# ifpen/wfcrl-env

Measured on AMD Instinct MI355X. Metric: farm_steps_per_sec, higher is better.
Workload: dtype f32

## Files before the change

### wfcrl-env_amd/csrc/wf_kernels_ll.hip

```cpp
#include <hip/hip_runtime.h>

#include <cstring>
#include <mutex>
#include <type_traits>
#include <utility>

#include "wf_kernel_common.h"

#ifndef WF_LL_PART
#define WF_LL_PART 0
#endif

namespace {

template <class F, int... I>
__device__ __forceinline__ void static_for_impl(F&& f, std::integer_sequence<int, I...>) {
  (f(std::integral_constant<int, I>{}), ...);
}
template <int N, class F>
__device__ __forceinline__ void static_for(F&& f) {
  static_for_impl(f, std::make_integer_sequence<int, N>{});
}

__device__ __forceinline__ void sincos_yaw(float x, float& s, float& c) {
  const float x2 = x * x;
  s = x * fmaf(x2, fmaf(x2, fmaf(x2, fmaf(x2, 2.7557319e-6f, -1.9841270e-4f), 8.3333333e-3f), -1.6666667e-1f), 1.0f);
  c = fmaf(x2, fmaf(x2, fmaf(x2, fmaf(x2, fmaf(x2, -2.7557319e-7f, 2.4801587e-5f), -1.3888889e-3f), 4.1666667e-2f), -0.5f), 1.0f);
  if (__any(fabsf(x) > 0.8f)) {
    float s2, c2;
    sincosf(x, &s2, &c2);
    s = (fabsf(x) > 0.8f) ? s2 : s;
    c = (fabsf(x) > 0.8f) ? c2 : c;
  }
}

template <int G>
__device__ __forceinline__ float wave_max(float v) {
  auto dpp = [](float x, auto ctrl, auto rows) {
    return __int_as_float(__builtin_amdgcn_update_dpp(__float_as_int(x), __float_as_int(x), decltype(ctrl)::value, decltype(rows)::value, 0xf, false));
  };
  using I = std::integral_constant<int, 0>;
  (void)sizeof(I);
  if constexpr (G < 2) v = fmaxf(v, dpp(v, std::integral_constant<int, 0xB1>{}, std::integral_constant<int, 0xf>{}));
  if constexpr (G < 4) v = fmaxf(v, dpp(v, std::integral_constant<int, 0x4E>{}, std::integral_constant<int, 0xf>{}));
  if constexpr (G < 8) v = fmaxf(v, dpp(v, std::integral_constant<int, 0x141>{}, std::integral_constant<int, 0xf>{}));
  if constexpr (G < 16) v = fmaxf(v, dpp(v, std::integral_constant<int, 0x140>{}, std::integral_constant<int, 0xf>{}));
  v = fmaxf(v, dpp(v, std::integral_constant<int, 0x142>{}, std::integral_constant<int, 0xa>{}));
  v = fmaxf(v, dpp(v, std::integral_constant<int, 0x143>{}, std::integral_constant<int, 0xc>{}));
  return __int_as_float(__builtin_amdgcn_readlane(__float_as_int(v), 63));
}

template <int G>
__device__ __forceinline__ float sub_max(float v) {
  auto dpp = [](float x, auto ctrl) {
    return __int_as_float(__builtin_amdgcn_update_dpp(__float_as_int(x), __float_as_int(x), decltype(ctrl)::value, 0xf, 0xf, false));
  };
  static_assert(G >= 2 && G <= 8, "sub_max: lanes per farm");
  if constexpr (G < 4) v = fmaxf(v, dpp(v, std::integral_constant<int, 0x4E>{}));
  if constexpr (G < 8) v = fmaxf(v, dpp(v, std::integral_constant<int, 0x124>{}));
  v = fmaxf(v, dpp(v, std::integral_constant<int, 0x128>{}));
  v = fmaxf(v, __shfl_xor(v, 16));
  v = fmaxf(v, __shfl_xor(v, 32));
  return v;
}

template <int G, int OS>
__device__ __forceinline__ float group_bcast(float v, int gbase) {
  if constexpr (G == 2) {
    return __int_as_float(__builtin_amdgcn_update_dpp(__float_as_int(v), __float_as_int(v), OS | (OS << 2) | ((2 + OS) << 4) | ((2 + OS) << 6), 0xf, 0xf, false));
  } else if constexpr (G == 4) {
    return __int_as_float(__builtin_amdgcn_update_dpp(__float_as_int(v), __float_as_int(v), OS * 0x55, 0xf, 0xf, false));
  } else {
    return __shfl(v, gbase + OS);
  }
}

struct SrcLog {
  float Gy, Gwt, sy0d, sz0d;
  float sM, tan_th0, sy0v, snw;
  float kdef, x0d, kyd, pj;
  float x0v, kyv, ch_pref, ix0v;
  float inv_s0d, d0;
};
struct ColdRec { float4 a, b, c; };
static_assert(WF_LOG_HOT_FLOATS == 2 && WF_LOG_COLD_FLOATS == 12, "source log record");
struct WfLogSide { float TI0, TI1, TI2, dTI; };
struct SrcB { float ubar, ct, a, Gwr, Gy, Gwt; unsigned risk; };
struct SrcD { SrcLog Sc; WfLogSide X; bool split; float x0num_d, pfac, b2om_d; };

}

#if WF_LL_PART != 1
__global__ void wf_pair_table_ll_kernel(const WfPairConsts pc, int G, const double* __restrict__ gx,
                                        const double* __restrict__ gy, float* __restrict__ tab, size_t group_floats,
                                        int* __restrict__ cross_tie, int* __restrict__ own_ok, int own_mode, double reach0,
                                        double reach_k) {
  const int i = blockIdx.x, t = threadIdx.x, grp = blockIdx.y;
  const int nblk = (pc.N + G - 1) / G;
  if (t >= nblk * G) return;
  gx += (size_t)grp * pc.N;
  gy += (size_t)grp * pc.N;
  const int J = t / G;
  if (own_mode == 1 && i >= J * G && i < t && t < pc.N) {
    const double dx = gx[t] - gx[i], dy = gy[t] - gy[i];
    if (dx <= 0.0 || fabs(dy) < reach0 + reach_k * dx) own_ok[(size_t)grp * nblk + J] = 0;
  }
  if (i >= (J + 1) * G) {
    if (t < pc.N && gx[t] - gx[i] >= 0.0) atomicOr(&cross_tie[grp], 1);
    return;
  }
  float* o = tab + (size_t)grp * group_floats + wf_ll_block_offset(J, pc.N, G) + ((size_t)i * G + (t - J * G)) * WF_PAIR_STRIDE;
  wf_pair_record(pc, gx, gy, i, t, o);
}

extern "C" size_t wfk_ll_table_floats(int N, int G) { return wf_ll_block_offset((N + G - 1) / G, N, G); }

extern "C" hipError_t wfk_launch_pair_table_ll(const WfPairConsts* pc, int G, int n_groups, const double* gx, const double* gy,
                                               float* tab, int* cross_tie, int* own_ok, int own_mode, double reach0,
                                               double reach_k, hipStream_t s) {
  const int nblk = (pc->N + G - 1) / G;
  const int threads = ((nblk * G + 63) / 64) * 64;
  hipError_t e = hipMemsetAsync(cross_tie, 0, sizeof(int) * (size_t)n_groups, s);
  if (e != hipSuccess) return e;
  e = hipMemsetD32Async((hipDeviceptr_t)own_ok, own_mode ? 1 : 0, (size_t)n_groups * nblk, s);
  if (e != hipSuccess) return e;
  hipLaunchKernelGGL(wf_pair_table_ll_kernel, dim3(pc->N, n_groups), dim3(threads), 0, s, *pc, G, gx, gy, tab,
                     wfk_ll_table_floats(pc->N, G), cross_tie, own_ok, own_mode, reach0, reach_k);
  return hipGetLastError();
}
#else
extern "C" size_t wfk_ll_table_floats(int N, int G);
#endif

#ifdef WF_LL_STAMP
static __device__ unsigned long long wf_ll_stamp[16];
#define WF_T(v) const unsigned long long v = __builtin_readcyclecounter()
#define WF_ACC(k, a, b) st_acc[k] += (b) - (a)
#else
#define WF_T(v)
#define WF_ACC(k, a, b)
#endif
template <int G, int S, bool UWS, bool TAB, bool MC1, int WPB, bool VEER = false, bool OCC2 = false>
__global__ __launch_bounds__(64 * WPB, ((S == 1 && !OCC2) ? 3 : 2) * 4 / WPB) void wf_step_ll_kernel(
    const WfConsts c, const WfTables* __restrict__ tab, const int* __restrict__ gidx, const double* __restrict__ ws_in,
    const double* __restrict__ wd_in, int wind_stride, const float* __restrict__ yaw_in, float* __restrict__ o_power,
    float* __restrict__ o_ws, float* __restrict__ o_wd, float* __restrict__ o_load, int B, const WfEnvArgs ea,
    const float* __restrict__ ll_tab, size_t group_floats, const int* __restrict__ cross_tie, float* __restrict__ src_log,
    size_t log_cold_offset, size_t log_side_offset, int n_pad, const WfGroupArgs ga, const double* __restrict__ gx,
    const double* __restrict__ gy, const int* __restrict__ own_ok) {
  constexpr int EPW = 64 / G;
  constexpr int GS = G * S;
  constexpr int CH = 64 / GS;
  constexpr bool STAGE = TAB && !VEER && GS <= CH;
  constexpr int CHUNK_FLOATS = TAB ? 64 * WF_PAIR_STRIDE : 4;
  __shared__ TableLds T;
  __shared__ __attribute__((aligned(16))) float prow[2][CHUNK_FLOATS];
  __shared__ unsigned risk_lds[WPB][EPW];
  __shared__ int env_lds[WPB][EPW];
  extern __shared__ __attribute__((aligned(16))) float yaw_lds[];

  if (ga.res_zero && blockIdx.x == 0 && threadIdx.x == 0) *ga.res_zero = 0;
  int grp = 0;
  if (ga.blk_group) {
    grp = ga.blk_group[(blockIdx.x * (WPB * EPW)) / ga.blk_unit];
    if (grp < 0) return;
    grp = (grp + ga.shift) % ga.mod;
  }
  if constexpr (TAB) {
    if (cross_tie[grp]) return;
    ll_tab += (size_t)grp * group_floats;
  }

  auto stage_chunk = [&](int q) {
    const char* g0 = reinterpret_cast<const char*>(ll_tab) + (size_t)q * (CHUNK_FLOATS * 4);
    char* l0 = reinterpret_cast<char*>(&prow[q & 1][0]);
    for (int ch = (int)(threadIdx.x >> 6); ch < CHUNK_FLOATS * 4 / 1024; ch += WPB)
      lds_dma16(g0 + ch * 1024 + (threadIdx.x & 63) * 16, l0 + ch * 1024, false);
  };
  if constexpr (TAB) stage_chunk(0);
  for (int k = threadIdx.x; k < WF_TABLE_PAD; k += blockDim.x) {
    T.knot[k] = tab->knot[k];
    T.ct[k] = tab->ct[k];
    T.cts[k] = tab->ct_slope[k];
    T.pw[k] = tab->pw[k];
    T.pws[k] = tab->pw_slope[k];
  }
  for (int k = threadIdx.x; k < WF_BUCKETS; k += blockDim.x) T.bucket[k] = tab->bucket[k];

  const int lane = threadIdx.x & 63;
  const int wave = threadIdx.x >> 6;
  const int sub = lane & (G - 1);
  const int gbase = lane & ~(G - 1);
  const int eiw = lane / G;
  const int slot = (blockIdx.x * WPB + wave) * EPW + eiw;
  int env_raw = slot + ga.env_base;
  if (ga.perm) env_raw = ga.perm[env_raw];
  bool env_ok = env_raw >= 0 && env_raw < (ga.env_end ? ga.env_end : B);
  const int env = env_ok ? env_raw : (B - 1);
  if constexpr (!TAB) env_ok = env_ok && !cross_tie[env];
  if (sub == 0) risk_lds[wave][eiw] = 0u;
  const int N = c.N;
  const int nblk = (N + GS - 1) / GS;

  auto uni = [](float v) { return UWS ? __int_as_float(__builtin_amdgcn_readfirstlane(__float_as_int(v))) : v; };
  const float ws = uni((float)ws_in[(size_t)env * wind_stride]);
  const double wd_d = fmod(wd_in[(size_t)env * wind_stride], 360.0);
  const float wd = uni((float)(wd_d < 0.0 ? wd_d + 360.0 : wd_d));
  const float Ui[3] = {uni(ws * c.shearf[0]), uni(ws * c.shearf[1]), uni(ws * c.shearf[2])};
  const float offk = c.off[2] * kGs;
  const float U02c = uni(Ui[0] * Ui[0] * Ui[0] + Ui[2] * Ui[2] * Ui[2]), U1c = uni(Ui[1] * Ui[1] * Ui[1]);
  auto cube_sum = [&](const float* e) {
    if constexpr (VEER) {
      float m = 0.0f;
#pragma unroll
      for (int j = 0; j < 3; ++j)
#pragma unroll
        for (int k = 0; k < 3; ++k) {
          const float u = Ui[k] * (1.0f - fsqrt(e[3 * j + k]));
          m = fmaf(u * u, u, m);
        }
      return m;
    } else {
      float fe = 0.0f, fc = 0.0f;
#pragma unroll
      for (int j = 0; j < 3; ++j) {
        const float ue = 1.0f - fsqrt(e[2 * j]), uc = 1.0f - fsqrt(e[2 * j + 1]);
        fe = fmaf(ue * ue, ue, fe);
        fc = fmaf(uc * uc, uc, fc);
      }
      return fmaf(U02c, fe, U1c * fc);
    }
  };
  const float ovh = 0.5f * c.guard_inv;
  const float ovs[3] = {uni(ovh * Ui[0] * c.inv_overlap_thr), uni(ovh * Ui[1] * c.inv_overlap_thr), uni(ovh * Ui[2] * c.inv_overlap_thr)};
  const float ovc = 0.5f - ovh;

  const size_t gofs = TAB ? (size_t)grp * N : (size_t)env * N;
  const size_t yofs = (size_t)env * N;
  const bool env_mode = ea.yaw_state != nullptr;
  int moves_new = 0;
  if (env_mode && ea.action) moves_new = ea.moves[env] + 1;
  if (sub == 0) env_lds[wave][eiw] = env_ok ? env : -1 - env;
  if (env_mode && ea.action) {
    int f = 0, o = lane;
    while (o >= N) { o -= N; ++f; }
    while (f < EPW) {
      const int e_raw = env_lds[wave][f];
      const bool okf = e_raw >= 0;
      const int e = okf ? e_raw : -1 - e_raw;
      const size_t oi = (size_t)e * N + o;
      float yw = ea.yaw_state[oi];
      float a = ea.action[oi];
      float acc = ea.acc[oi];
      const float frac = __fdiv_rn(__fdiv_rn(__fdiv_rn(acc, ea.rate), (float)(ea.moves[e] + 1)), ea.dt);
      if (frac >= ea.budget) a = 0.0f;
      if (ea.discrete) a = (a - 1.0f) * ea.yaw_step;
      if (!ea.discrete) a = fminf(fmaxf(a, -ea.yaw_step), ea.yaw_step);
      yw = fminf(fmaxf(yw + a, ea.yaw_lo), ea.yaw_hi);
      acc += fabsf(a);
      if (okf) {
        ea.yaw_state[oi] = yw;
        ea.acc[oi] = acc;
        if (ea.yaw_out) ea.yaw_out[oi] = yw;
      }
      o += 64;
      while (o >= N) { o -= N; ++f; }
    }
  }
  const float* const yaw_src = (env_mode ? ea.yaw_state : yaw_in) + yofs;
  const bool yaw_fresh = env_mode && ea.action;
  auto load_yaw = [&](int o) { return yaw_fresh ? __hip_atomic_load(yaw_src + o, __ATOMIC_RELAXED, __HIP_MEMORY_SCOPE_AGENT) : yaw_src[o]; };
  if (env_mode && ea.action && sub == 0 && env_ok) ea.moves[env] = moves_new;
  if constexpr (TAB) wf_dma_wait();
  __syncthreads();

  constexpr int NE = VEER ? 9 : 6;
  float esq[S][NE], V[S][9], W[S][9], TI[S][3];
  const float amb0 = fsqrt(c.amb2);

  auto apply_tab = [&](auto PP, const float4* pr, float Gy, float Gwt) {
    constexpr int p = decltype(PP)::value;
#pragma unroll
    for (int j = 0; j < 3; ++j) {
      const float4 cf[3] = {pr[3 * j], pr[3 * j + 1], pr[3 * j + 2]};
#pragma unroll
      for (int k = 0; k < 3; ++k) {
        const int q = j * 3 + k;
        V[p][q] = fmaf(Gwt, cf[k].y, fmaf(Gy, cf[k].x, V[p][q]));
        const float ww = fmaf(Gwt, cf[k].w, Gy * cf[k].z);
        W[p][q] += fmaxf(ww, 0.0f);
      }
    }
  };

  auto apply_tab_ratio = [&](auto PP, const float4* pr, float rho, float Gwt) {
    constexpr int p = decltype(PP)::value;
    const float lim = copysignf(__builtin_inff(), Gwt);
#pragma unroll
    for (int q = 0; q < 9; ++q) {
      const float4 cf = pr[q];
      V[p][q] = fmaf(Gwt, fmaf(rho, cf.x, cf.y), V[p][q]);
      W[p][q] = fmaf(Gwt, __builtin_amdgcn_fmed3f(fmaf(rho, cf.z, cf.w), 0.0f, lim), W[p][q]);
    }
  };

  auto apply_fly = [&](auto PP, float dx, float dy, float Gy, float Gwt) {
    constexpr int p = decltype(PP)::value;
    const float Gt = c.gam_top * Gy, Gb = -c.gam_bot * Gy;
    float dec[3];
#pragma unroll
    for (int k = 0; k < 3; ++k) dec[k] = frcp(fmaf(c.decay_a[k], dx, 1.0f));
#pragma unroll
    for (int j = 0; j < 3; ++j) {
      const float yL = dy + c.yoff[j];
      const float yL2 = yL * yL;
      const float Ey = fexp2(-yL2 * c.exp_c);
      float A[3] = {0.0f, 0.0f, 0.0f}, Bw[3] = {0.0f, 0.0f, 0.0f};
#pragma unroll
      for (int mi = 0; mi < 7; ++mi) {
        float tr = fmaf(-Ey, c.ez[mi], 1.0f) * frcp(yL2 + c.zc2[mi]);
        if (mi == 3) {
          const float ts = fmaf(yL2 + c.zc2[3], c.m_half_inv_eps4, c.inv_eps2);
          tr = (yL2 < c.yl2_small) ? ts : tr;
        }
// ... 327 lines not shown
  };
  auto src_far_bound = [&](const SrcD& d, const float* TIs, float& k6, float& b6, float& n6) {
    const SrcLog& Sc = d.Sc;
    const float s0 = VEER ? c.sz0v : Sc.sy0v;
    float kyv_m = Sc.kyv, bb = fmaf(-Sc.kyv, Sc.x0v, s0);
    float db = fabsf(Sc.tan_th0 * Sc.x0d) + 2.2f * fabsf(Sc.pj);
    if (__any(d.split)) {
      const float TImax = fmaxf(TIs[0], fmaxf(TIs[1], TIs[2])), TImin = fminf(TIs[0], fminf(TIs[1], TIs[2]));
      const float x0d_m = d.x0num_d * frcp(fmaf(c.alpha4_d, TImin, d.b2om_d));
      const float pj_m = d.pfac * frcp(fmaf(c.ka_d, TImin, c.kb_d));
      kyv_m = fmaf(c.ka, TImax + d.X.dTI, c.kb);
      bb = d.split ? s0 : bb;
      db = fabsf(Sc.tan_th0 * x0d_m) + 2.2f * fabsf(pj_m);
    }
    const float dbo = db + c.off[2];
    k6 = c.far_k * kyv_m;
    b6 = fmaf(c.far_k, bb, dbo);
    n6 = fmaf(c.far_k, fmaxf(Sc.snw, s0), dbo);
  };
  auto within_bound = [&](const float4 bnd, float dx, float dy) {
    return fabsf(dy) < fmaxf(fmaf(bnd.x, dx, bnd.y), bnd.z) + fabsf(fmaf(c.bd, dx, c.ad));
  };
  int oidx[S], oidx_nx[S], oidx_n2[S];
  float yaw_nx[S];
#pragma unroll
  for (int p = 0; p < S; ++p) {
    oidx_nx[p] = gidx[gofs + min(p * G + sub, N - 1)];
    oidx_n2[p] = gidx[gofs + min(GS + p * G + sub, N - 1)];
  }
#pragma unroll
  for (int p = 0; p < S; ++p) yaw_nx[p] = load_yaw(oidx_nx[p]);
  for (int J = 0; J < nblk; ++J) {
    int tt[S];
    bool tvalid[S];
    float yaw_t[S], sg_t[S], cg_t[S];
    double xt_d[TAB ? 1 : S] = {}, yt_d[TAB ? 1 : S] = {};
#pragma unroll
    for (int p = 0; p < S; ++p) {
      tt[p] = J * GS + p * G + sub;
      tvalid[p] = tt[p] < N;
      if constexpr (!TAB) {
        xt_d[p] = tvalid[p] ? gx[gofs + tt[p]] : -1.0e300;
        yt_d[p] = gy[gofs + (tvalid[p] ? tt[p] : 0)];
      }
#pragma unroll
      for (int k = 0; k < 9; ++k) { V[p][k] = 0.0f; W[p][k] = 0.0f; }
#pragma unroll
      for (int k = 0; k < NE; ++k) esq[p][k] = 0.0f;
#pragma unroll
      for (int j = 0; j < 3; ++j) TI[p][j] = amb0;
      oidx[p] = oidx_nx[p];
      yaw_t[p] = yaw_nx[p];
      oidx_nx[p] = oidx_n2[p];
      oidx_n2[p] = gidx[gofs + min(tt[p] + 2 * GS, N - 1)];
      yaw_nx[p] = load_yaw(oidx_nx[p]);
      sincos_yaw(yaw_t[p] * kDeg2Rad, sg_t[p], cg_t[p]);
    }

    const int first_own = J * GS;
    const int n_src = min(N, first_own + GS);
    const int n_chunks = (n_src + CH - 1) / CH;
    float2 hot_nx = make_float2(0.0f, 0.0f);
    ColdRec cold_nx = {};
    double xs_nx = 0.0, ys_nx = 0.0;
    if (first_own > 0) {
      if constexpr (!TAB) {
        hot_nx = load_hot(0);
        cold_nx = load_cold(0);
        xs_nx = gx[gofs];
        ys_nx = gy[gofs];
      }
    }

    auto fly_record = [&](auto PP, double xi, double yi) {
      constexpr int p = decltype(PP)::value;
      constexpr int q = TAB ? 0 : p;
      float4 r;
      r.x = (float)(xt_d[q] - xi);
      r.y = (float)(yt_d[q] - yi);
      r.z = (xt_d[q] <= xi + c.fifteenD_d) ? 1.0f : 0.0f;
      r.w = __int_as_float((xt_d[q] > xi + 0.1) ? 8 : 0);
      return r;
    };

    auto own_source = [&](auto PS, int i, const float* recs) {
      constexpr int ps = decltype(PS)::value;
      const int src = gbase + ((i - first_own) - ps * G);
      __builtin_amdgcn_s_setprio(3);
      WF_T(so_0);
      float vsum = 0.0f;
#pragma unroll
      for (int k2 = 0; k2 < 9; ++k2) vsum += V[ps][k2];
      const float m3 = __shfl(cube_sum(esq[ps]), src);
      const float Vmean = __shfl(vsum, src) * (1.0f / 9.0f);
      float TIs[3];
#pragma unroll
      for (int j = 0; j < 3; ++j) TIs[j] = __shfl(TI[ps][j], src);
      const float yaw_i = __shfl(yaw_t[ps], src);
      const float cg = __shfl(cg_t[ps], src), sg = __shfl(sg_t[ps], src);
      WF_T(so_1);
      WF_ACC(6, so_0, so_1);
      const SrcB Bs = src_part_b(m3, cg, sg);
      if (Bs.risk) atomicOr(&risk_lds[wave][eiw], Bs.risk);
      WF_T(so_2);
      WF_ACC(7, so_1, so_2);
      float4 ex[S];
      double xi_d = 0.0, yi_d = 0.0;
      if constexpr (!TAB) {
        xi_d = gx[gofs + i];
        yi_d = gy[gofs + i];
      }
      auto pass1_slot = [&](auto PP) {
        constexpr int p = decltype(PP)::value;
        if constexpr (TAB) {
          const float* rec = recs + (p * G + sub) * WF_PAIR_STRIDE;
          ex[p] = *reinterpret_cast<const float4*>(rec + WF_PAIR_DX);
          const bool act1 = (p > ps) ? tvalid[p] : (ex[p].x >= 0.0f);
          if (p >= ps || __any(act1)) {
            if (act1) apply_tab(PP, reinterpret_cast<const float4*>(rec), Bs.Gy, Bs.Gwt);
          }
        } else {
          ex[p] = fly_record(PP, xi_d, yi_d);
          const bool act1 = (p > ps) ? tvalid[p] : (ex[p].x >= 0.0f);
          if (p >= ps || __any(act1)) {
            if (act1) apply_fly(PP, ex[p].x, ex[p].y, Bs.Gy, Bs.Gwt);
          }
        }
      };
      static_for<S>(pass1_slot);
      WF_T(so_3);
      WF_ACC(8, so_2, so_3);
      float vbar = 0.0f, wbar = 0.0f;
#pragma unroll
      for (int k2 = 0; k2 < 9; ++k2) { vbar += V[ps][k2]; wbar += W[ps][k2]; }
      vbar = __shfl(vbar, src) * (1.0f / 9.0f);
      wbar = __shfl(wbar, src) * (1.0f / 9.0f);
      const SrcD Ds = src_part_d(Bs, Vmean, vbar, wbar, TIs, yaw_i, cg, sg, [](bool f) { return __any(f) != 0; });
      const SrcLog& Sc = Ds.Sc;
      const WfLogSide& X = Ds.X;
      if (lane == src) {
#pragma unroll
        for (int j = 0; j < 3; ++j) TI[ps][j] = fmaxf(TI[ps][j] + X.dTI, amb0);
      }
      if (J + 1 < nblk) {
        if (sub == 0) log_store(i, Ds);
        float k6, b6, n6;
        src_far_bound(Ds, TIs, k6, b6, n6);
        k6 = wave_max<G>(k6);
        b6 = wave_max<G>(b6);
        n6 = wave_max<G>(n6);
        if (!c.far_on) { k6 = 0.0f; b6 = 0.0f; n6 = 3.0e38f; }
        if (lane == 0) bndL[i] = make_float4(k6, b6, n6, 0.0f);
      }
      WF_T(so_4);
      WF_ACC(9, so_3, so_4);
      const float xs_[4] = {X.TI0, X.TI1, X.TI2, X.dTI};
      static_for<S>([&](auto PP) {
        constexpr int p = decltype(PP)::value;
        if constexpr (p == ps) pass2(PP, Sc, xs_, false, ex[p], ex[p].x > 0.0f, yt_d[TAB ? 0 : p], yi_d);
        else if constexpr (p > ps) pass2(PP, Sc, xs_, false, ex[p], tvalid[p], yt_d[TAB ? 0 : p], yi_d);
      });
      WF_T(so_5);
      WF_ACC(10, so_4, so_5);
      __builtin_amdgcn_s_setprio(0);
    };

    auto own_stage = [&](const float* buf, int k0, int nm) -> bool {
      if constexpr (STAGE) {
        __builtin_amdgcn_s_setprio(3);
        int ln = lane;
        asm volatile("" : "+v"(ln));
        const int sub = ln & (G - 1), gbase = ln & ~(G - 1), eiw = ln / G;
        float2* const sv = saveL + ln;
#pragma unroll
        for (int p = 0; p < S; ++p)
#pragma unroll
          for (int k2 = 0; k2 < 9; ++k2) sv[(p * 9 + k2) * 64] = make_float2(V[p][k2], W[p][k2]);
        SrcB Bm[S];
        float Vmean[S], vbar[S], wbar[S];
#pragma unroll
        for (int p = 0; p < S; ++p) {
          Bm[p] = src_part_b(cube_sum(esq[p]), cg_t[p], sg_t[p]);
          Vmean[p] = 0.0f; vbar[p] = 0.0f; wbar[p] = 0.0f;
        }
        static_for<GS>([&](auto MM) {
          constexpr int m = decltype(MM)::value;
          constexpr int ps = m / G, os = m % G;
          if (m < nm) {
            float vs = 0.0f;
#pragma unroll
            for (int k2 = 0; k2 < 9; ++k2) vs += V[ps][k2];
            Vmean[ps] = (sub == os) ? vs * (1.0f / 9.0f) : Vmean[ps];
            const float Gy = group_bcast<G, os>(Bm[ps].Gy, gbase), Gwt = group_bcast<G, os>(Bm[ps].Gwt, gbase);
            const float* recs = buf + ((k0 + m) * GS) * WF_PAIR_STRIDE;
            static_for<S>([&](auto PP) {
              constexpr int p = decltype(PP)::value;
              const float* rec = recs + (p * G + sub) * WF_PAIR_STRIDE;
              const bool act1 = (p > ps) ? tvalid[p] : (rec[WF_PAIR_DX] >= 0.0f);
              if (p >= ps || __any(act1)) {
                if (act1) apply_tab(PP, reinterpret_cast<const float4*>(rec), Gy, Gwt);
              }
            });
            float vb = 0.0f, wb = 0.0f;
#pragma unroll
            for (int k2 = 0; k2 < 9; ++k2) { vb += V[ps][k2]; wb += W[ps][k2]; }
            vbar[ps] = (sub == os) ? vb * (1.0f / 9.0f) : vbar[ps];
            wbar[ps] = (sub == os) ? wb * (1.0f / 9.0f) : wbar[ps];
          }
        });
        unsigned long long sub_lanes = 0ull;
#pragma unroll
        for (int e = 0; e < EPW; ++e) sub_lanes |= 1ull << (e * G);
        sub_lanes <<= sub;
        float dTI[S];
#pragma unroll
        for (int p = 0; p < S; ++p) {
          const float TIs[3] = {TI[p][0], TI[p][1], TI[p][2]};
          const SrcD Dm = src_part_d(Bm[p], Vmean[p], vbar[p], wbar[p], TIs, yaw_t[p], cg_t[p], sg_t[p],
                                     [&](bool f) { return (__ballot(f) & sub_lanes) != 0ull; });
          dTI[p] = Dm.X.dTI;
          int it = tt[p];
          asm volatile("" : "+v"(it));
          if (J + 1 < nblk && tvalid[p]) log_store(it, Dm);
          float k6, b6, n6;
          src_far_bound(Dm, TIs, k6, b6, n6);
          k6 = sub_max<G>(k6);
          b6 = sub_max<G>(b6);
          n6 = sub_max<G>(n6);
          if (!c.far_on) { k6 = 0.0f; b6 = 0.0f; n6 = 3.0e38f; }
          if (ln < G && tvalid[p]) bndL[tt[p]] = make_float4(k6, b6, n6, 0.0f);
        }
        __builtin_amdgcn_fence(__ATOMIC_RELEASE, "wavefront");
        __builtin_amdgcn_wave_barrier();
        __builtin_amdgcn_fence(__ATOMIC_ACQUIRE, "wavefront");
        bool reach = false;
        {
          const int ma = ln / GS, mb = ln % GS;
          if (ma < mb && mb < nm) {
            const float2 e = *reinterpret_cast<const float2*>(buf + ((k0 + ma) * GS + mb) * WF_PAIR_STRIDE + WF_PAIR_DX);
            reach = within_bound(bndL[first_own + ma], e.x, e.y);
          }
        }
        const bool stands = __ballot(reach) == 0ull;
#ifdef WF_LL_STAMP
        st_acc[12] += 1ull;
        st_acc[13] += stands ? 0ull : 1ull;
#endif
        if (stands) {
#pragma unroll
          for (int p = 0; p < S; ++p) {
            if (tvalid[p] && Bm[p].risk) atomicOr(&risk_lds[wave][eiw], Bm[p].risk);
#pragma unroll
            for (int j = 0; j < 3; ++j) TI[p][j] = fmaxf(TI[p][j] + dTI[p], amb0);
          }
        } else {
#pragma unroll
          for (int p = 0; p < S; ++p)
#pragma unroll
            for (int k2 = 0; k2 < 9; ++k2) {
              const float2 vw = sv[(p * 9 + k2) * 64];
              V[p][k2] = vw.x; W[p][k2] = vw.y;
            }
        }
        __builtin_amdgcn_s_setprio(0);
        return stands;
      } else {
        return false;
      }
    };
    bool spec_J = false;
    if constexpr (STAGE) {
      if (own_ok) spec_J = own_ok[(size_t)grp * nblk + J] != 0;
    }

    for (int cq = 0; cq < n_chunks; ++cq, ++q) {
      if constexpr (TAB) {
        if (cq == 0 && first_own > 0) wf_dma_wait();
        if (cq + 1 < n_chunks || J + 1 < nblk) stage_chunk(q + 1);
        if (cq + 1 < n_chunks && (cq + 1) * CH < first_own) stage_hot(q + 1, (cq + 1) * CH);
      }
      const float* buf = &prow[q & 1][0];
      const int i0 = cq * CH;
      const int k_log = min(max(first_own - i0, 0), CH);
      const int k_end = min(n_src - i0, CH);
      WF_T(st_a);
      if constexpr (TAB) {
        if (k_log > 0) {
          unsigned long long near_bits, pair_bits;
          {
            const int kk = lane / GS, rr = lane % GS;
            const float2 e = *reinterpret_cast<const float2*>(buf + (kk * GS + rr) * WF_PAIR_STRIDE + WF_PAIR_DX);
            const float4 bnd = bndL[min(i0 + kk, n_pad - 1)];
            pair_bits = __ballot(kk < k_log && (J * GS + rr) < N && within_bound(bnd, e.x, e.y));
            near_bits = pair_bits;
#pragma unroll
            for (int sh = 1; sh < GS; sh <<= 1) near_bits |= near_bits >> sh;
            unsigned long long rep = 0ull;
#pragma unroll
            for (int kq = 0; kq < CH; ++kq) rep |= 1ull << (kq * GS);
            near_bits &= rep;
          }
          ColdRec cold_nx = {};
          if (near_bits) cold_nx = load_cold(i0 + (__builtin_ctzll(near_bits) / GS));
          static_assert(GS % 2 == 0 && CH % 2 == 0, "logged sources come in pairs");
#pragma unroll 1
          for (int k = 0; k < k_log; k += 2) {
            const float4 hot2 = hotL[(q & 1) * HOT_F4 + (k >> 1) * EPW + eiw];
            float4 cf[S][9];
#pragma unroll
            for (int p = 0; p < S; ++p)
#pragma unroll
              for (int qq = 0; qq < 9; ++qq)
                cf[p][qq] = *reinterpret_cast<const float4*>(buf + (k * GS + p * G + sub) * WF_PAIR_STRIDE + 4 * qq);
            static_for<S>([&](auto PP) { apply_tab_ratio(PP, cf[decltype(PP)::value], hot2.x, hot2.y); });
#pragma unroll
            for (int p = 0; p < S; ++p)
#pragma unroll
              for (int qq = 0; qq < 9; ++qq)
                cf[p][qq] = *reinterpret_cast<const float4*>(buf + ((k + 1) * GS + p * G + sub) * WF_PAIR_STRIDE + 4 * qq);
            static_for<S>([&](auto PP) { apply_tab_ratio(PP, cf[decltype(PP)::value], hot2.z, hot2.w); });
          }
          WF_T(st_ab);
          WF_ACC(11, st_a, st_ab);
          auto near_step = [&](int k, const ColdRec& cold, ColdRec& nxt) {
            const int i = i0 + k;
            float4 exs[S];
#pragma unroll
            for (int p = 0; p < S; ++p)
              exs[p] = *reinterpret_cast<const float4*>(buf + (k * GS + p * G + sub) * WF_PAIR_STRIDE + WF_PAIR_DX);
            asm volatile("" ::: "memory");
#ifdef WF_EXP_NOCOLD
            nxt = cold;
#else
            nxt = load_cold(near_bits ? i0 + (__builtin_ctzll(near_bits) / GS) : i);
#endif
            const SrcLog Sl = unpack(make_float2(0.0f, 0.0f), cold);
            const float* side = logx + (size_t)i * WF_LOG_SIDE_FLOATS;
            static_for<S>([&](auto PP) {
              constexpr int p = decltype(PP)::value;
              if ((pair_bits >> (k * GS + p * G)) & ((1ull << G) - 1ull)) pass2(PP, Sl, side, true, exs[p], tvalid[p]);
            });
          };
          ColdRec cold_b = {};
          __builtin_amdgcn_s_setprio(1);
#pragma unroll 1
          while (near_bits) {
            const int k0 = __builtin_ctzll(near_bits) / GS;
            near_bits &= near_bits - 1ull;
            near_step(k0, cold_nx, cold_b);
            if (!near_bits) break;
            const int k1 = __builtin_ctzll(near_bits) / GS;
            near_bits &= near_bits - 1ull;
            near_step(k1, cold_b, cold_nx);
          }
          __builtin_amdgcn_s_setprio(0);
        }
      } else {
#pragma unroll 1
        for (int k = 0; k < k_log; ++k) {
          const int i = i0 + k;
          const float2 hot = hot_nx;
          const ColdRec cold = cold_nx;
          const int inx = min(i + 1, first_own - 1);
          const float* side = logx + (size_t)i * WF_LOG_SIDE_FLOATS;
          const double xs_d = xs_nx, ys_d = ys_nx;
          hot_nx = load_hot(inx);
          cold_nx = load_cold(inx);
          xs_nx = gx[gofs + inx];
          ys_nx = gy[gofs + inx];
          const float4 bnd = bndL[i];
          float4 exr[S];
          int nr = 0;
          static_for<S>([&](auto PP) {
            constexpr int p = decltype(PP)::value;
            exr[p] = fly_record(PP, xs_d, ys_d);
            nr |= (int)tvalid[p] & (int)within_bound(bnd, exr[p].x, exr[p].y);
          });
          const bool near = __any(nr != 0);
          const SrcLog Sl = unpack(hot, cold);
          static_for<S>([&](auto PP) {
            constexpr int p = decltype(PP)::value;
            if (tvalid[p]) apply_fly(PP, exr[p].x, exr[p].y, hot.x * hot.y, hot.y);
            if (near) pass2(PP, Sl, side, true, exr[p], tvalid[p], yt_d[TAB ? 0 : p], ys_d);
          });
        }
      }
      WF_T(st_b);
      WF_ACC(0, st_a, st_b);
      bool staged = false;
      if constexpr (STAGE) {
        if (spec_J && k_log < k_end) staged = own_stage(buf, k_log, k_end - k_log);
      }
#pragma unroll 1
      for (int k = staged ? k_end : k_log; k < k_end; ++k) {
        const int i = i0 + k;
        const float* recs = buf + (k * GS) * WF_PAIR_STRIDE;
        const int slot_of_source = (i - first_own) / G;
        static_for<S>([&](auto PS) {
          if (slot_of_source == decltype(PS)::value) own_source(PS, i, recs);
        });
      }
      WF_T(st_c);
      WF_ACC(1, st_b, st_c);
      if constexpr (TAB) {
        wf_dma_wait();
        __syncthreads();
      }
      WF_T(st_d);
      WF_ACC(2, st_c, st_d);
    }
    if constexpr (TAB) {
      if (J + 1 < nblk) stage_hot(q, 0);
    }
    WF_T(st_e);

#pragma unroll
    for (int p = 0; p < S; ++p) {
      if (!tvalid[p]) continue;
      const int o = oidx[p];
      float U[9], m3 = 0.0f, mu = 0.0f, mv = 0.0f, mw = 0.0f, adir = 0.0f;
#pragma unroll
      for (int j = 0; j < 3; ++j) {
        if constexpr (VEER) {
#pragma unroll
          for (int k = 0; k < 3; ++k) U[3 * j + k] = Ui[k] * (1.0f - fsqrt(esq[p][3 * j + k]));
        } else {
          const float ue = 1.0f - fsqrt(esq[p][2 * j]), uc = 1.0f - fsqrt(esq[p][2 * j + 1]);
          U[3 * j] = Ui[0] * ue; U[3 * j + 1] = Ui[1] * uc; U[3 * j + 2] = Ui[2] * ue;
        }
      }
#pragma unroll
      for (int k = 0; k < 9; ++k) {
        m3 = fmaf(U[k] * U[k], U[k], m3);
        mu += U[k]; mv += V[p][k]; mw += W[p][k];
      }
      if (o_wd) {
        bool small = true;
        float rr[9];
#pragma unroll
        for (int k = 0; k < 9; ++k) {
          rr[k] = V[p][k] * frcp(U[k]);
          small = small && (U[k] > 0.0f) && (fabsf(rr[k]) <= 0.25f);
        }
        if (__all(small)) {
#pragma unroll
          for (int k = 0; k < 9; ++k) adir += atan_small(rr[k]);
        } else {
#pragma unroll
          for (int k = 0; k < 9; ++k) adir += atan2f(V[p][k], U[k]);
        }
      }
      mu *= (1.0f / 9.0f); mv *= (1.0f / 9.0f); mw *= (1.0f / 9.0f);
      float su = 0.0f, sv = 0.0f, sw = 0.0f;
#pragma unroll
      for (int k = 0; k < 9; ++k) {
        const float du = U[k] - mu, dv = V[p][k] - mv, dw = W[p][k] - mw;
        su = fmaf(du, du, su); sv = fmaf(dv, dv, sv); sw = fmaf(dw, dw, sw);
      }
      const float wsp = fcbrt_pos(m3 * (1.0f / 9.0f));
      {
        float umin = U[0];
#pragma unroll
        for (int k = 1; k < 9; ++k) umin = fminf(umin, U[k]);
        if (!(umin > 0.0f)) atomicOr(&risk_lds[wave][eiw], (unsigned)WF_RISK_NEGATIVE_SPEED);
      }
      const float veff = c.dens_f * wsp * fexp2(c.pw * flog2(cg_t[p]));
      float pslope;
      const float pwr = c.rho * table_pw(c, T, veff, pslope);
      if (c.rho * fabsf(pslope) * veff > c.knee_kappa * fmaxf(pwr, 1.0e3f))
        atomicOr(&risk_lds[wave][eiw], (unsigned)WF_RISK_POWER_KNEE);
      float4 l;
      l.x = (TI[p][0] + TI[p][1] + TI[p][2]) * (1.0f / 3.0f);
      l.y = fsqrt(su * (1.0f / 9.0f));
      l.z = fsqrt(sv * (1.0f / 9.0f));
      l.w = fsqrt(sw * (1.0f / 9.0f));
      const bool real = o < n_real;
      psum += real ? pwr : 0.0f;
      lsum += real ? (l.x + l.y) + (l.z + l.w) : 0.0f;
      if (env_ok) {
        const size_t oo = yofs + o;
        if (o_power) o_power[oo] = real ? (ea.power_mw ? pwr * 1.0e-6f : pwr) : 0.0f;
        if (o_ws) o_ws[oo] = real ? wsp : 0.0f;
        if (o_wd) o_wd[oo] = real ? wd - adir * (kRad2Deg / 9.0f) : 0.0f;
        if (o_load) reinterpret_cast<float4*>(o_load)[oo] = real ? l : make_float4(0.0f, 0.0f, 0.0f, 0.0f);
      }
    }
    WF_T(st_f);
    WF_ACC(3, st_e, st_f);
  }
#ifdef WF_LL_STAMP
  if (lane == 0) {
    st_acc[4] = __builtin_readcyclecounter() - st_begin;
    for (int k = 0; k < 5; ++k) atomicAdd(&wf_ll_stamp[k], st_acc[k]);
    atomicAdd(&wf_ll_stamp[5], 1ull);
    for (int k = 6; k < 14; ++k) atomicAdd(&wf_ll_stamp[k], st_acc[k]);
  }
#endif

  if (ga.risk_flags && sub == 0 && env_ok) {
    const int rf = (int)risk_lds[wave][eiw];
    ga.risk_flags[env] = rf;
    if (ga.res_list) {
      ga.flags_raw[env] = rf;
      if (rf & ga.res_mask) ga.res_list[atomicAdd(ga.res_count, 1)] = env;
    }
  }
  if (ea.reward) {
#pragma unroll
    for (int w = G / 2; w >= 1; w >>= 1) {
      psum += __shfl_xor(psum, w);
      lsum += __shfl_xor(lsum, w);
    }
    if (sub == 0 && env_ok) {
      const float invN = __fdiv_rn(1.0f, (float)n_real);
      const float wr = ea.ws_prev ? (float)ea.ws_prev[env] : ws;
      const float r = psum * invN * 1.0e-3f * frcp(wr * wr * wr) - ea.load_coef * lsum * invN * 0.25f;
      ea.reward[env] = r;
    }
  }
}

constexpr int kLLWaves = 4;

template <int G, int S, bool TAB, bool MC1, bool VEER = false>
static hipError_t launch_ll(const WfConsts* c, const WfTables* tab, const int* gidx, const double* ws, const double* wd,
                            int wind_stride, const float* yaw, float* power, float* o_ws, float* o_wd, float* load, int B,
                            const WfEnvArgs* env, const float* ll_tab, const int* cross_tie, float* src_log, size_t log_records,
                            const WfGroupArgs* grp, const double* gx, const double* gy, const int* own_ok, hipStream_t s) {
  constexpr int fpb = kLLWaves * (64 / G);
  WfGroupArgs ga = *grp;
  const int n_farms = ga.env_end ? ga.env_end - ga.env_base : B;
  const int grid = ga.blk_group ? (ga.n_slots + fpb - 1) / fpb : (n_farms + fpb - 1) / fpb;
  WfConsts cc = *c;
  WfEnvArgs ea;
  if (env) ea = *env; else memset(&ea, 0, sizeof(ea));
  size_t group_floats = wfk_ll_table_floats(cc.N, G * S);
  int n_pad = ((cc.N + G * S - 1) / (G * S)) * (G * S);
  constexpr int hot_bytes = 32768 / (G * G * S) >= 1024 ? 32768 / (G * G * S) : 1024;
  size_t dyn_lds = sizeof(float4) * (size_t)kLLWaves * n_pad + (TAB ? (size_t)kLLWaves * 2 * hot_bytes : 0);
  size_t log_cold_offset = log_records * WF_LOG_HOT_FLOATS, log_side_offset = log_records * WF_LOG_FLOATS;
  void* args[] = {&cc, &tab, &gidx, &ws, &wd, &wind_stride, &yaw, &power, &o_ws, &o_wd, &load, &B, &ea, &ll_tab,
                  &group_floats, &cross_tie, &src_log, &log_cold_offset, &log_side_offset, &n_pad, &ga, &gx, &gy, &own_ok};
  const void* fn = (const void*)&wf_step_ll_kernel<G, S, false, TAB, MC1, kLLWaves, VEER>;
  if constexpr (TAB) {
    if (wind_stride == 0) fn = (const void*)&wf_step_ll_kernel<G, S, true, TAB, MC1, kLLWaves, VEER>;
  }
  if constexpr (S == 1 && (MC1 || !TAB) && !VEER) {
    static int n_cu_of[64] = {};
    int dev = 0, n_cu = 0;
    if (hipGetDevice(&dev) == hipSuccess && dev >= 0 && dev < 64) {
      n_cu = n_cu_of[dev];
      if (n_cu == 0 && hipDeviceGetAttribute(&n_cu, hipDeviceAttributeMultiprocessorCount, dev) == hipSuccess) n_cu_of[dev] = n_cu;
    }
    if (n_cu > 0 && grid <= 2 * n_cu)
      fn = wind_stride == 0 ? (const void*)&wf_step_ll_kernel<G, S, true, TAB, MC1, kLLWaves, VEER, true>
                            : (const void*)&wf_step_ll_kernel<G, S, false, TAB, MC1, kLLWaves, VEER, true>;
  }
  if (!(TAB && !VEER && G * S <= 64 / (G * S)) || !cc.far_on) own_ok = nullptr;
  if (own_ok) {
    const size_t save_wave = sizeof(float) * 18 * S * 64;
    const size_t save_bytes = save_wave > 2 * (size_t)hot_bytes ? (save_wave - 2 * (size_t)hot_bytes) * kLLWaves : 0;
    struct Occ { const void* fn; size_t lds; int keeps; };
    static Occ seen[16] = {};
    static int n_seen = 0;
    static std::mutex seen_mutex;
    std::lock_guard<std::mutex> lock(seen_mutex);
    int keeps = -1;
    for (int k = 0; k < n_seen; ++k)
      if (seen[k].fn == fn && seen[k].lds == dyn_lds) keeps = seen[k].keeps;
    if (keeps < 0) {
      int without = 0, with = 0;
      keeps = (hipOccupancyMaxActiveBlocksPerMultiprocessor(&without, fn, 64 * kLLWaves, dyn_lds) == hipSuccess &&
               hipOccupancyMaxActiveBlocksPerMultiprocessor(&with, fn, 64 * kLLWaves, dyn_lds + save_bytes) == hipSuccess && with >= without && with > 0) ? 1 : 0;
      if (n_seen < 16) seen[n_seen++] = Occ{fn, dyn_lds, keeps};
    }
    if (keeps) dyn_lds += save_bytes; else own_ok = nullptr;
  }
  return hipLaunchKernel(fn, dim3(grid), dim3(64 * kLLWaves), args, dyn_lds, s);
}

#if WF_LL_PART != 1
extern "C" int wfk_ll_farms_per_block(int G) { return kLLWaves * (64 / G); }
#endif
#if WF_LL_PART != 2
#ifdef WF_LL_STAMP
extern "C" int wfk_ll_stamps(unsigned long long* out, int reset) {
  hipError_t e = hipMemcpyFromSymbol(out, HIP_SYMBOL(wf_ll_stamp), sizeof(wf_ll_stamp));
  if (e == hipSuccess && reset) {
    unsigned long long z[16] = {};
    e = hipMemcpyToSymbol(HIP_SYMBOL(wf_ll_stamp), z, sizeof(z));
  }
  return (int)e;
}
#endif

#endif

#define WF_LL_DISPATCH(G_, S_, CALL) \
  if (G == G_ && S == S_) return CALL(G_, S_)
#define WF_LL_STEP_ARGS                                                                                                          \
  int G, int S, const WfConsts *c, const WfTables *tab, const int *gidx, const double *ws, const double *wd, int wind_stride,   \
      const float *yaw, float *power, float *o_ws, float *o_wd, float *load, int B, const WfEnvArgs *env, const float *ll_tab,    \
      const int *cross_tie, const int *own_ok, float *src_log, size_t log_records, const WfGroupArgs *grp, hipStream_t s
#define WF_LL_LAUNCH(G_, S_) launch_ll<G_, S_, true, true>(c, tab, gidx, ws, wd, wind_stride, yaw, power, o_ws, o_wd, load, B, env, ll_tab, cross_tie, src_log, log_records, grp, nullptr, nullptr, own_ok, s)
#if WF_LL_PART != 2
extern "C" hipError_t wfk_launch_step_ll_s2(WF_LL_STEP_ARGS) {
  WF_LL_DISPATCH(4, 2, WF_LL_LAUNCH);
  WF_LL_DISPATCH(2, 2, WF_LL_LAUNCH);
  return hipErrorInvalidValue;
}
extern "C" hipError_t wfk_ll_func_attributes_s2(int G, int S, int shared_speed, hipFuncAttributes* a) {
#define WF_LL_ATTR_S2(G_, S_) hipFuncGetAttributes(a, shared_speed ? (const void*)&wf_step_ll_kernel<G_, S_, true, true, true, kLLWaves> : (const void*)&wf_step_ll_kernel<G_, S_, false, true, true, kLLWaves>)
  WF_LL_DISPATCH(4, 2, WF_LL_ATTR_S2);
  WF_LL_DISPATCH(2, 2, WF_LL_ATTR_S2);
  return hipErrorInvalidValue;
}
#endif

#if WF_LL_PART != 1
extern "C" hipError_t wfk_launch_step_ll_s2(WF_LL_STEP_ARGS);
extern "C" hipError_t wfk_ll_func_attributes_s2(int G, int S, int shared_speed, hipFuncAttributes* a);
extern "C" hipError_t wfk_launch_step_ll(int G, int S, const WfConsts* c, const WfTables* tab, const int* gidx, const double* ws,
                                         const double* wd, int wind_stride, const float* yaw, float* power, float* o_ws,
                                         float* o_wd, float* load, int B, const WfEnvArgs* env, const float* ll_tab,
                                         const int* cross_tie, const int* own_ok, float* src_log, size_t log_records,
                                         const WfGroupArgs* grp, hipStream_t s) {
#define WF_LL_LAUNCH_VEER(G_, S_) launch_ll<G_, S_, true, true, true>(c, tab, gidx, ws, wd, wind_stride, yaw, power, o_ws, o_wd, load, B, env, ll_tab, cross_tie, src_log, log_records, grp, nullptr, nullptr, nullptr, s)
  if (c->veer_on) {
    WF_LL_DISPATCH(4, 1, WF_LL_LAUNCH_VEER);
    WF_LL_DISPATCH(4, 2, WF_LL_LAUNCH_VEER);
    WF_LL_DISPATCH(2, 2, WF_LL_LAUNCH_VEER);
    return hipErrorInvalidValue;
  }
  WF_LL_DISPATCH(4, 1, WF_LL_LAUNCH);
  WF_LL_DISPATCH(8, 1, WF_LL_LAUNCH);
  WF_LL_DISPATCH(16, 1, WF_LL_LAUNCH);
  if (S == 2) return wfk_launch_step_ll_s2(G, S, c, tab, gidx, ws, wd, wind_stride, yaw, power, o_ws, o_wd, load, B, env, ll_tab, cross_tie, own_ok, src_log, log_records, grp, s);
  return hipErrorInvalidValue;
}

extern "C" int wfk_ll_has_veer(int G, int S, int table) { return table ? ((G == 4 && S <= 2) || (G == 2 && S == 2)) : (G == 4 && S == 2); }

extern "C" int wfk_ll_has_fly(int G, int S) { return (G == 4 && S <= 2) || (G == 8 && S == 1) || (G == 2 && S == 2); }

extern "C" hipError_t wfk_launch_step_ll_fly(int G, int S, const WfConsts* c, const WfTables* tab, const int* gidx, const double* gx,
                                             const double* gy, const double* ws, const double* wd, const float* yaw,
                                             float* power, float* o_ws, float* o_wd, float* load, int B, const WfEnvArgs* env,
                                             const int* farm_tie, float* src_log, size_t log_records,
                                             const WfGroupArgs* grp, hipStream_t s) {
#define WF_LL_LAUNCH_FLY(G_, S_)                                                                                              \
  (c->mirror_core_n <= 1                                                                                                      \
       ? launch_ll<G_, S_, false, true>(c, tab, gidx, ws, wd, 1, yaw, power, o_ws, o_wd, load, B, env, nullptr, farm_tie, src_log, \
                                        log_records, grp, gx, gy, nullptr, s)                                                       \
       : launch_ll<G_, S_, false, false>(c, tab, gidx, ws, wd, 1, yaw, power, o_ws, o_wd, load, B, env, nullptr, farm_tie,      \
                                         src_log, log_records, grp, gx, gy, nullptr, s))
  if (c->veer_on) {
    if (G == 4 && S == 2)
      return launch_ll<4, 2, false, false, true>(c, tab, gidx, ws, wd, 1, yaw, power, o_ws, o_wd, load, B, env, nullptr, farm_tie, src_log,
                                                 log_records, grp, gx, gy, nullptr, s);
    return hipErrorInvalidValue;
  }
  WF_LL_DISPATCH(4, 2, WF_LL_LAUNCH_FLY);
  WF_LL_DISPATCH(2, 2, WF_LL_LAUNCH_FLY);
  WF_LL_DISPATCH(4, 1, WF_LL_LAUNCH_FLY);
  WF_LL_DISPATCH(8, 1, WF_LL_LAUNCH_FLY);
  return hipErrorInvalidValue;
}

extern "C" hipError_t wfk_ll_func_attributes_fly(int G, int S, int veer, int occ2, hipFuncAttributes* a) {
  if (veer) return (G == 4 && S == 2) ? hipFuncGetAttributes(a, (const void*)&wf_step_ll_kernel<4, 2, false, false, true, kLLWaves, true>) : hipErrorInvalidValue;
#define WF_LL_ATTR_FLY(G_, S_) hipFuncGetAttributes(a, (const void*)&wf_step_ll_kernel<G_, S_, false, false, true, kLLWaves>)
#define WF_LL_ATTR_FLY_OCC2(G_, S_) hipFuncGetAttributes(a, (const void*)&wf_step_ll_kernel<G_, S_, false, false, true, kLLWaves, false, true>)
  if (occ2) {
    WF_LL_DISPATCH(4, 1, WF_LL_ATTR_FLY_OCC2);
    WF_LL_DISPATCH(8, 1, WF_LL_ATTR_FLY_OCC2);
  }
  WF_LL_DISPATCH(4, 2, WF_LL_ATTR_FLY);
  WF_LL_DISPATCH(2, 2, WF_LL_ATTR_FLY);
  WF_LL_DISPATCH(4, 1, WF_LL_ATTR_FLY);
  WF_LL_DISPATCH(8, 1, WF_LL_ATTR_FLY);
  return hipErrorInvalidValue;
}

extern "C" hipError_t wfk_ll_func_attributes(int G, int S, int shared_speed, int table, int veer, int occ2, hipFuncAttributes* a) {
  if (!table) return wfk_ll_func_attributes_fly(G, S, veer, occ2, a);
#define WF_LL_ATTR_VEER(G_, S_) hipFuncGetAttributes(a, shared_speed ? (const void*)&wf_step_ll_kernel<G_, S_, true, true, true, kLLWaves, true> : (const void*)&wf_step_ll_kernel<G_, S_, false, true, true, kLLWaves, true>)
  if (veer) {
    WF_LL_DISPATCH(4, 1, WF_LL_ATTR_VEER);
    WF_LL_DISPATCH(4, 2, WF_LL_ATTR_VEER);
    WF_LL_DISPATCH(2, 2, WF_LL_ATTR_VEER);
    return hipErrorInvalidValue;
  }
#define WF_LL_ATTR(G_, S_) hipFuncGetAttributes(a, shared_speed ? (const void*)&wf_step_ll_kernel<G_, S_, true, true, true, kLLWaves> : (const void*)&wf_step_ll_kernel<G_, S_, false, true, true, kLLWaves>)
#define WF_LL_ATTR_OCC2(G_, S_) hipFuncGetAttributes(a, shared_speed ? (const void*)&wf_step_ll_kernel<G_, S_, true, true, true, kLLWaves, false, true> : (const void*)&wf_step_ll_kernel<G_, S_, false, true, true, kLLWaves, false, true>)
  if (occ2) {
    WF_LL_DISPATCH(4, 1, WF_LL_ATTR_OCC2);
    WF_LL_DISPATCH(8, 1, WF_LL_ATTR_OCC2);
    WF_LL_DISPATCH(16, 1, WF_LL_ATTR_OCC2);
  }
  WF_LL_DISPATCH(4, 1, WF_LL_ATTR);
  WF_LL_DISPATCH(8, 1, WF_LL_ATTR);
  WF_LL_DISPATCH(16, 1, WF_LL_ATTR);
  if (S == 2) return wfk_ll_func_attributes_s2(G, S, shared_speed, a);
  return hipErrorInvalidValue;
}
#endif
```

Baseline: 83.59 million.

## Add staged LDS waitcnt, deeper cold-record prefetch, and chunk vmcnt switches

Measured after the change: 86.39 million (median of 6 runs). 3.3% higher.

```diff
diff --git a/wfcrl-env_amd/csrc/wf_kernels_ll.hip b/wfcrl-env_amd/csrc/wf_kernels_ll.hip
--- a/wfcrl-env_amd/csrc/wf_kernels_ll.hip
+++ b/wfcrl-env_amd/csrc/wf_kernels_ll.hip
@@ -10,6 +10,16 @@
 #ifndef WF_LL_PART
 #define WF_LL_PART 0
 #endif
+#ifndef WF_LL_CHUNK_VMCNT
+#define WF_LL_CHUNK_VMCNT (WF_LL_PART == 1)
+#endif
+#ifndef WF_LL_TRANS_WAIT
+#define WF_LL_TRANS_WAIT (WF_LL_PART == 1 ? 2 : 0)
+#endif
+#ifndef WF_LL_COLD_DEPTH
+#define WF_LL_COLD_DEPTH 1
+#endif
+static_assert(WF_LL_TRANS_WAIT >= 0 && WF_LL_TRANS_WAIT <= 2 && (WF_LL_COLD_DEPTH == 1 || WF_LL_COLD_DEPTH == 2), "replay A/B switches");
 
 namespace {
 
@@ -20,6 +30,14 @@
 template <int N, class F>
 __device__ __forceinline__ void static_for(F&& f) {
   static_for_impl(f, std::make_integer_sequence<int, N>{});
+}
+
+template <int LGKM>
+__device__ __forceinline__ void lds_wait_here() {
+  static_assert(LGKM >= 0 && LGKM <= 15, "lgkmcnt has four bits");
+  __builtin_amdgcn_sched_barrier(0);
+  __builtin_amdgcn_s_waitcnt(0xC07F | (LGKM << 8));
+  __builtin_amdgcn_sched_barrier(0);
 }
 
 __device__ __forceinline__ void sincos_yaw(float x, float& s, float& c) {
@@ -953,11 +971,16 @@
           }
           ColdRec cold_nx = {};
           if (near_bits) cold_nx = load_cold(i0 + (__builtin_ctzll(near_bits) / GS));
+#if WF_LL_COLD_DEPTH == 2
+          ColdRec cold_b = {}, cold_c = {};
+          if (near_bits & (near_bits - 1ull)) cold_b = load_cold(i0 + (__builtin_ctzll(near_bits & (near_bits - 1ull)) / GS));
+#endif
           static_assert(GS % 2 == 0 && CH % 2 == 0, "logged sources come in pairs");
 #pragma unroll 1
           for (int k = 0; k < k_log; k += 2) {
             const float4 hot2 = hotL[(q & 1) * HOT_F4 + (k >> 1) * EPW + eiw];
             float4 cf[S][9];
+#if WF_LL_TRANS_WAIT == 0
 #pragma unroll
             for (int p = 0; p < S; ++p)
 #pragma unroll
@@ -970,6 +993,25 @@
               for (int qq = 0; qq < 9; ++qq)
                 cf[p][qq] = *reinterpret_cast<const float4*>(buf + ((k + 1) * GS + p * G + sub) * WF_PAIR_STRIDE + 4 * qq);
             static_for<S>([&](auto PP) { apply_tab_ratio(PP, cf[decltype(PP)::value], hot2.z, hot2.w); });
+#else
+            auto one_source = [&](int kk, float rho, float Gwt) {
+              static_for<S>([&](auto PP) {
+                constexpr int p = decltype(PP)::value;
+#pragma unroll
+                for (int qq = 0; qq < 9; ++qq)
+                  cf[p][qq] = *reinterpret_cast<const float4*>(buf + (kk * GS + p * G + sub) * WF_PAIR_STRIDE + 4 * qq);
+                if constexpr (WF_LL_TRANS_WAIT == 2 && p + 1 < S) __builtin_amdgcn_sched_barrier(0);
+              });
+              static_for<S>([&](auto PP) {
+                constexpr int p = decltype(PP)::value;
+                if constexpr (WF_LL_TRANS_WAIT == 2) lds_wait_here<9 * (S - 1 - p)>();
+                else if constexpr (p == 0) lds_wait_here<0>();
+                apply_tab_ratio(PP, cf[p], rho, Gwt);
+              });
+            };
+            one_source(k, hot2.x, hot2.y);
+            one_source(k + 1, hot2.z, hot2.w);
+#endif
           }
           WF_T(st_ab);
           WF_ACC(11, st_a, st_ab);
@@ -982,6 +1024,9 @@
             asm volatile("" ::: "memory");
 #ifdef WF_EXP_NOCOLD
             nxt = cold;
+#elif WF_LL_COLD_DEPTH == 2
+            const unsigned long long ahead2 = near_bits & (near_bits - 1ull);
+            nxt = load_cold(ahead2 ? i0 + (__builtin_ctzll(ahead2) / GS) : i);
 #else
             nxt = load_cold(near_bits ? i0 + (__builtin_ctzll(near_bits) / GS) : i);
 #endif
@@ -992,8 +1037,26 @@
               if ((pair_bits >> (k * GS + p * G)) & ((1ull << G) - 1ull)) pass2(PP, Sl, side, true, exs[p], tvalid[p]);
             });
           };
+#if WF_LL_COLD_DEPTH == 1
           ColdRec cold_b = {};
+#endif
           __builtin_amdgcn_s_setprio(1);
+#if WF_LL_COLD_DEPTH == 2
+#pragma unroll 1
+          while (near_bits) {
+            const int k0 = __builtin_ctzll(near_bits) / GS;
+            near_bits &= near_bits - 1ull;
+            near_step(k0, cold_nx, cold_c);
+            if (!near_bits) break;
+            const int k1 = __builtin_ctzll(near_bits) / GS;
+            near_bits &= near_bits - 1ull;
+            near_step(k1, cold_b, cold_nx);
+            if (!near_bits) break;
+            const int k2 = __builtin_ctzll(near_bits) / GS;
+            near_bits &= near_bits - 1ull;
+            near_step(k2, cold_c, cold_b);
+          }
+#else
 #pragma unroll 1
           while (near_bits) {
             const int k0 = __builtin_ctzll(near_bits) / GS;
@@ -1004,6 +1067,7 @@
             near_bits &= near_bits - 1ull;
             near_step(k1, cold_b, cold_nx);
           }
+#endif
           __builtin_amdgcn_s_setprio(0);
         }
       } else {
@@ -1055,6 +1119,9 @@
       WF_ACC(1, st_b, st_c);
       if constexpr (TAB) {
         wf_dma_wait();
+#if WF_LL_CHUNK_VMCNT
+        __builtin_amdgcn_s_waitcnt(0x0F70);
+#endif
         __syncthreads();
       }
       WF_T(st_d);
```
